# mkofinas/aether

Hardware: AMD Instinct MI355X
Metric: edge-messages/sec (forward, electrostatic N=20 batch=128 per GPU) (higher is better)
Workload: dtype f32; 1 GPU; electrostatic-2d-N20-B128; num_dims=2, nodes_per_graph=20, graphs_per_gpu=128, edges_per_gpu=48640, hidden=64, launch=hipgraph (10 steps per replay), parallelism=graphs sharded over 1 rank(s), no forward collective

## Files before the change

aether_amd/csrc/common.h:

```cpp
#pragma once
#include <hip/hip_runtime.h>
#include <cstdint>
#include <type_traits>
#include "../../include/aether_hip.h"

namespace {

typedef float f32x4 __attribute__((ext_vector_type(4)));
typedef float f32x2 __attribute__((ext_vector_type(2)));

constexpr int H = AETHER_HIDDEN;
constexpr int LDW = H + 8;
constexpr int FPAD = 32;
constexpr int LDF = FPAD + 8;
constexpr int LDST = H + 4;
constexpr float PI_F = 3.14159274101257324f;
constexpr float TWO_PI_F = 6.28318548202514648f;
constexpr float EPS_F = 1e-7f;

__device__ __forceinline__ void lds_barrier() { asm volatile("s_waitcnt lgkmcnt(0)\n\ts_barrier" ::: "memory"); }

__device__ __forceinline__ f32x4 mfma16(float a, float b, f32x4 c) {
    return __builtin_amdgcn_mfma_f32_16x16x4f32(a, b, c, 0, 0, 0);
}
// ... 121 lines not shown
    }
    const int frag = (mb * KBN + kb) * 64 + m + 16 * qq;
    constexpr int TERM = MBN * KBN * 64;
    *reinterpret_cast<f16x4*>(img + (frag) * 4 + half * 2) = h;
    *reinterpret_cast<f16x4*>(img + (TERM + frag) * 4 + half * 2) = l;
}

__device__ __forceinline__ unsigned wave_max_bits(float m) {
    int v = __float_as_int(m);
#define AETHER_DPP_MAX(CTRL) { const int o = __builtin_amdgcn_update_dpp(0, v, CTRL, 0xf, 0xf, true); v = o > v ? o : v; }
    AETHER_DPP_MAX(0x111) AETHER_DPP_MAX(0x112) AETHER_DPP_MAX(0x114) AETHER_DPP_MAX(0x118) AETHER_DPP_MAX(0x142) AETHER_DPP_MAX(0x143)
#undef AETHER_DPP_MAX
    return (unsigned)__builtin_amdgcn_readlane(v, 63);
}
__device__ __forceinline__ unsigned wave_max_exponent(float m) { return (wave_max_bits(m) >> 23) & 255u; }
struct SplitScale { bool on; float s, inv_s; };
__device__ __forceinline__ float absmax4(float m, const f32x4 v) {
#ifdef AETHER_SPLIT_PARENT_FORMS
    return fmaxf(fmaxf(m, fmaxf(fabsf(v[0]), fabsf(v[1]))), fmaxf(fabsf(v[2]), fabsf(v[3])));
#else
    m = fmaxf(fmaxf(m, fabsf(v[0])), fabsf(v[1]));
    return fmaxf(fmaxf(m, fabsf(v[2])), fabsf(v[3]));
#endif
}
template <int N>
__device__ __forceinline__ SplitScale split_scale_of(const f32x4 (&act)[N]) {
    float m = 0.0f;
#pragma unroll
    for (int b = 0; b < N; ++b) m = absmax4(m, act[b]);
    const bool big = __builtin_amdgcn_ballot_w64(m >= 32768.0f) != 0ull;
    const bool some = __builtin_amdgcn_ballot_w64(m >= 0.015625f) != 0ull;
    const bool any = __builtin_amdgcn_ballot_w64(m > 0.0f) != 0ull;
    SplitScale r;
    r.on = big || (any && !some);
    r.s = 1.0f; r.inv_s = 1.0f;
    if (r.on) {
        const unsigned E = wave_max_exponent(m);
        int sh = 140 - (int)E;
        sh = sh > 40 ? 40 : (sh < -40 ? -40 : sh);
        r.s = __int_as_float((127 + sh) << 23);
        r.inv_s = __int_as_float((127 - sh) << 23);
    }
    return r;
}

template <int MBN, int KBN>
__device__ __forceinline__ void gemm_split_core(const f16x8* __restrict__ w, const f32x4 (&act)[2 * KBN], f32x4 (&acc)[MBN], int lane,
                                                f16x8 (&xh)[KBN], f16x8 (&xl)[KBN]) {
    constexpr int TERM = MBN * KBN * 64;
#pragma unroll
    for (int kb = 0; kb < KBN; ++kb) {
        split8(act[2 * kb], act[2 * kb + 1], xh[kb], xl[kb]);
#pragma unroll
        for (int mb = 0; mb < MBN; ++mb) {
            const int frag = (mb * KBN + kb) * 64 + lane;
            const f16x8 wh = w[frag], wl = w[TERM + frag];
            acc[mb] = __builtin_amdgcn_mfma_f32_16x16x32_f16(wl, xh[kb], acc[mb], 0, 0, 0);
            acc[mb] = __builtin_amdgcn_mfma_f32_16x16x32_f16(wh, xl[kb], acc[mb], 0, 0, 0);
            acc[mb] = __builtin_amdgcn_mfma_f32_16x16x32_f16(wh, xh[kb], acc[mb], 0, 0, 0);
        }
    }
}
template <int MBN, int KBN>
__device__ __forceinline__ SplitScale gemm_split_keep(const float* __restrict__ img, const f32x4 (&act)[2 * KBN], f32x4 (&acc)[MBN],
                                                      int lane, f16x8 (&xh)[KBN], f16x8 (&xl)[KBN]) {
    const SplitScale sc = split_scale_of(act);
    f32x4 x[2 * KBN];
#pragma unroll
    for (int b = 0; b < 2 * KBN; ++b) x[b] = act[b];
    if (sc.on) {
#pragma unroll
        for (int b = 0; b < 2 * KBN; ++b) x[b] = x[b] * sc.s;
#pragma unroll
        for (int mb = 0; mb < MBN; ++mb) acc[mb] = acc[mb] * sc.s;
    }
    gemm_split_core<MBN, KBN>(reinterpret_cast<const f16x8*>(img), x, acc, lane, xh, xl);
    if (sc.on) {
#pragma unroll
        for (int mb = 0; mb < MBN; ++mb) acc[mb] = acc[mb] * sc.inv_s;
    }
    return sc;
}
template <int MBN, int KBN>
__device__ __forceinline__ void gemm_split(const float* __restrict__ img, const f32x4 (&act)[2 * KBN], f32x4 (&acc)[MBN],
                                           int lane) {
    f16x8 xh[KBN], xl[KBN];
    (void)gemm_split_keep<MBN, KBN>(img, act, acc, lane, xh, xl);
}

template <int MBN, int KBN>
__device__ __forceinline__ void gemm_split_paired(const float* __restrict__ img, const f32x4 (&act)[2 * KBN], f32x4 (&acc)[MBN], int lane) {
    static_assert(MBN % 2 == 0, "row blocks go in pairs");
    constexpr int TERM = MBN * KBN * 64, NG = KBN * (MBN / 2);
    const f16x8* w = reinterpret_cast<const f16x8*>(img);
    const SplitScale sc = split_scale_of(act);
    f32x4 x[2 * KBN];
#pragma unroll
    for (int b = 0; b < 2 * KBN; ++b) x[b] = act[b];
    if (sc.on) {
#pragma unroll
        for (int b = 0; b < 2 * KBN; ++b) x[b] = x[b] * sc.s;
#pragma unroll
        for (int mb = 0; mb < MBN; ++mb) acc[mb] = acc[mb] * sc.s;
    }
    auto frag = [&](int g, int j, bool lo) -> f16x8 {
        const int kb = g / (MBN / 2), mb = 2 * (g % (MBN / 2)) + j;
        return w[(lo ? TERM : 0) + (mb * KBN + kb) * 64 + lane];
    };
    f16x8 xh[KBN], xl[KBN];
    f16x8 wl0 = frag(0, 0, true), wl1 = frag(0, 1, true), wh0 = frag(0, 0, false), wh1 = frag(0, 1, false);
    split8(x[0], x[1], xh[0], xl[0]);
#pragma unroll
    for (int g = 0; g < NG; ++g) {
        const int kb = g / (MBN / 2), m0 = 2 * (g % (MBN / 2)), m1 = m0 + 1;
        __builtin_amdgcn_sched_barrier(0);
        acc[m0] = __builtin_amdgcn_mfma_f32_16x16x32_f16(wl0, xh[kb], acc[m0], 0, 0, 0);
        acc[m1] = __builtin_amdgcn_mfma_f32_16x16x32_f16(wl1, xh[kb], acc[m1], 0, 0, 0);
        __builtin_amdgcn_sched_barrier(0);
        if (g + 1 < NG) { wl0 = frag(g + 1, 0, true); wl1 = frag(g + 1, 1, true); }
        if (g + 1 < NG && (g + 1) % (MBN / 2) == 0) split8(x[2 * (kb + 1)], x[2 * (kb + 1) + 1], xh[kb + 1], xl[kb + 1]);
        acc[m0] = __builtin_amdgcn_mfma_f32_16x16x32_f16(wh0, xl[kb], acc[m0], 0, 0, 0);
        acc[m1] = __builtin_amdgcn_mfma_f32_16x16x32_f16(wh1, xl[kb], acc[m1], 0, 0, 0);
        acc[m0] = __builtin_amdgcn_mfma_f32_16x16x32_f16(wh0, xh[kb], acc[m0], 0, 0, 0);
        acc[m1] = __builtin_amdgcn_mfma_f32_16x16x32_f16(wh1, xh[kb], acc[m1], 0, 0, 0);
        __builtin_amdgcn_sched_barrier(0);
        if (g + 1 < NG) { wh0 = frag(g + 1, 0, false); wh1 = frag(g + 1, 1, false); }
    }
    if (sc.on) {
#pragma unroll
        for (int mb = 0; mb < MBN; ++mb) acc[mb] = acc[mb] * sc.inv_s;
    }
}

template <int KBN>
__device__ __forceinline__ f32x4 gemm_split_regs(const f16x8 (&wh)[KBN], const f16x8 (&wl)[KBN], const f32x4 (&act)[2 * KBN], f32x4 acc) {
    const SplitScale sc = split_scale_of(act);
    f32x4 x[2 * KBN];
#pragma unroll
    for (int b = 0; b < 2 * KBN; ++b) x[b] = act[b];
    if (sc.on) {
#pragma unroll
        for (int b = 0; b < 2 * KBN; ++b) x[b] = x[b] * sc.s;
        acc = acc * sc.s;
    }
#pragma unroll
    for (int kb = 0; kb < KBN; ++kb) {
        f16x8 xh, xl;
        split8(x[2 * kb], x[2 * kb + 1], xh, xl);
        acc = __builtin_amdgcn_mfma_f32_16x16x32_f16(wl[kb], xh, acc, 0, 0, 0);
        acc = __builtin_amdgcn_mfma_f32_16x16x32_f16(wh[kb], xl, acc, 0, 0, 0);
        acc = __builtin_amdgcn_mfma_f32_16x16x32_f16(wh[kb], xh, acc, 0, 0, 0);
    }
    if (sc.on) acc = acc * sc.inv_s;
    return acc;
}
template <int MBN, int KBN>
__device__ __forceinline__ void load_split_frags(const float* __restrict__ img, int mb, int lane, f16x8 (&wh)[KBN], f16x8 (&wl)[KBN]) {
    const f16x8* w = reinterpret_cast<const f16x8*>(img) + __builtin_amdgcn_readfirstlane(mb) * (KBN * 64);
    constexpr int TERM = MBN * KBN * 64;
#pragma unroll
    for (int kb = 0; kb < KBN; ++kb) {
        wh[kb] = w[kb * 64 + lane];
        wl[kb] = w[TERM + kb * 64 + lane];
    }
}

template <int KBN, int BLK>
__device__ __forceinline__ void split_T_issue(unsigned base, u32x2 (&lo)[2], u32x2 (&hi)[2]) {
    constexpr int TERM_BYTES = 4 * KBN * 64 * 16, OB = 2 * KBN, mp = BLK / OB, ob = BLK % OB;
#pragma unroll
    for (int t = 0; t < 2; ++t)
        asm volatile("ds_read_b64_tr_b16 %0, %2 offset:%3\n\tds_read_b64_tr_b16 %1, %2 offset:%4"
                     : "=&v"(lo[t]), "=&v"(hi[t])
                     : "v"(base), "n"(t * TERM_BYTES + (((2 * mp) * KBN + (ob >> 1)) * 64) * 16 + (ob & 1) * 8),
                       "n"(t * TERM_BYTES + (((2 * mp + 1) * KBN + (ob >> 1)) * 64) * 16 + (ob & 1) * 8)
                     : "memory");
}
template <bool LAST>
__device__ __forceinline__ void split_T_consume(u32x2 (&lo)[2], u32x2 (&hi)[2], const f16x8 xh, const f16x8 xl, f32x4& acc) {
    if constexpr (LAST)
        asm volatile("s_waitcnt lgkmcnt(0)" : "+v"(lo[0]), "+v"(hi[0]), "+v"(lo[1]), "+v"(hi[1]));
    else
        asm volatile("s_waitcnt lgkmcnt(4)" : "+v"(lo[0]), "+v"(hi[0]), "+v"(lo[1]), "+v"(hi[1]));
    f16x8 w[2];
#pragma unroll
    for (int t = 0; t < 2; ++t) {
        const u32x4 v = {lo[t][0], lo[t][1], hi[t][0], hi[t][1]};
        w[t] = __builtin_bit_cast(f16x8, v);
    }
    const f16x8 wh = w[0], wl = w[1];
    acc = __builtin_amdgcn_mfma_f32_16x16x32_f16(wl, xh, acc, 0, 0, 0);
    acc = __builtin_amdgcn_mfma_f32_16x16x32_f16(wh, xl, acc, 0, 0, 0);
    acc = __builtin_amdgcn_mfma_f32_16x16x32_f16(wh, xh, acc, 0, 0, 0);
}
template <int KBN, int BLK>
__device__ __forceinline__ void split_T_step(unsigned base, u32x2 (&lo)[2][2], u32x2 (&hi)[2][2], const f16x8 (&xh)[2],
                                             const f16x8 (&xl)[2], f32x4 (&acc)[2 * KBN]) {
    constexpr int OB = 2 * KBN, NBLK = 2 * OB, mp = BLK / OB, ob = BLK % OB;
    if constexpr (BLK + 1 < NBLK) split_T_issue<KBN, BLK + 1>(base, lo[(BLK + 1) & 1], hi[(BLK + 1) & 1]);
    split_T_consume<BLK + 1 == NBLK>(lo[BLK & 1], hi[BLK & 1], xh[mp], xl[mp], acc[ob]);
    if constexpr (BLK + 1 < NBLK) split_T_step<KBN, BLK + 1>(base, lo, hi, xh, xl, acc);
}
template <int KBN>
__device__ __forceinline__ SplitScale gemm_split_T_keep(const float* __restrict__ img, const f32x4 (&act)[4], f32x4 (&acc)[2 * KBN],
                                                        int lane, f16x8 (&xh)[2], f16x8 (&xl)[2]) {
    const int g = lane >> 4, r = (lane & 15) >> 2, p = lane & 3;
    const unsigned base = (unsigned)(size_t)(__attribute__((address_space(3))) const char*)img + ((4 * g + r) + 16 * p) * 16;
    const SplitScale sc = split_scale_of(act);
    f32x4 x[4];
#pragma unroll
    for (int b = 0; b < 4; ++b) x[b] = act[b];
    if (sc.on) {
#pragma unroll
        for (int b = 0; b < 4; ++b) x[b] = x[b] * sc.s;
    }
    split8(x[0], x[1], xh[0], xl[0]);
    split8(x[2], x[3], xh[1], xl[1]);
    u32x2 lo[2][2], hi[2][2];
    split_T_issue<KBN, 0>(base, lo[0], hi[0]);
    split_T_step<KBN, 0>(base, lo, hi, xh, xl, acc);
    if (sc.on) {
#pragma unroll
        for (int ob = 0; ob < 2 * KBN; ++ob) acc[ob] = acc[ob] * sc.inv_s;
    }
    return sc;
}
template <int KBN>
__device__ __forceinline__ void gemm_split_T(const float* __restrict__ img, const f32x4 (&act)[4], f32x4 (&acc)[2 * KBN],
                                             int lane) {
    f16x8 xh[2], xl[2];
    (void)gemm_split_T_keep<KBN>(img, act, acc, lane, xh, xl);
}

template <int MBN, int KBN>
__device__ __forceinline__ void gemm_split_pieces(const float* __restrict__ img, const f16x8 (&xh)[KBN], const f16x8 (&xl)[KBN],
                                                  const SplitScale sc, f32x4 (&acc)[MBN], int lane) {
    constexpr int TERM = MBN * KBN * 64;
    const f16x8* w = reinterpret_cast<const f16x8*>(img);
    if (sc.on) {
#pragma unroll
        for (int mb = 0; mb < MBN; ++mb) acc[mb] = acc[mb] * own_reg(sc.s);
    }
#pragma unroll
    for (int kb = 0; kb < KBN; ++kb)
#pragma unroll
        for (int mb = 0; mb < MBN; ++mb) {
            const int frag = (mb * KBN + kb) * 64 + lane;
            const f16x8 wh = w[frag], wl = w[TERM + frag];
            acc[mb] = __builtin_amdgcn_mfma_f32_16x16x32_f16(wl, xh[kb], acc[mb], 0, 0, 0);
            acc[mb] = __builtin_amdgcn_mfma_f32_16x16x32_f16(wh, xl[kb], acc[mb], 0, 0, 0);
            acc[mb] = __builtin_amdgcn_mfma_f32_16x16x32_f16(wh, xh[kb], acc[mb], 0, 0, 0);
        }
    if (sc.on) {
#pragma unroll
        for (int mb = 0; mb < MBN; ++mb) acc[mb] = acc[mb] * own_reg(sc.inv_s);
    }
}
template <int KBN>
__device__ __forceinline__ SplitScale split_tile(const f32x4 (&act)[2 * KBN], f16x8 (&xh)[KBN], f16x8 (&xl)[KBN]) {
    const SplitScale sc = split_scale_of(act);
#pragma unroll
    for (int kb = 0; kb < KBN; ++kb) {
        if (sc.on) split8(act[2 * kb] * own_reg(sc.s), act[2 * kb + 1] * own_reg(sc.s), xh[kb], xl[kb]);
        else split8(act[2 * kb], act[2 * kb + 1], xh[kb], xl[kb]);
    }
    return sc;
}

constexpr int FB_RH = 2 * LDST;
constexpr int FB_PLANE = 16 * FB_RH;
static_assert(2 * FB_PLANE == 16 * LDST * 4, "the two pieces take the room of the fp32 rows");
template <int KBN>
__device__ __forceinline__ void fb_stage_pieces(float* arr, int i, int q, const f16x8 (&xh)[KBN], const f16x8 (&xl)[KBN]) {
    char* row = reinterpret_cast<char*>(arr) + i * FB_RH + 8 * q;
#pragma unroll
    for (int kb = 0; kb < KBN; ++kb) {
        const u32x4 h = __builtin_bit_cast(u32x4, xh[kb]), l = __builtin_bit_cast(u32x4, xl[kb]);
        *reinterpret_cast<u32x2*>(row + 64 * kb) = u32x2{h[0], h[1]};
        *reinterpret_cast<u32x2*>(row + 64 * kb + 32) = u32x2{h[2], h[3]};
        *reinterpret_cast<u32x2*>(row + FB_PLANE + 64 * kb) = u32x2{l[0], l[1]};
        *reinterpret_cast<u32x2*>(row + FB_PLANE + 64 * kb + 32) = u32x2{l[2], l[3]};
    }
}
__device__ __forceinline__ unsigned fb_tr_lane_offset(int lane) {
    const int q = lane >> 4, c = lane & 15;
    return (unsigned)((4 * q + (c >> 2)) * FB_RH + 8 * (c & 3));
}
__device__ __forceinline__ unsigned fb_lds_addr(const float* p) { return (unsigned)(size_t)(__attribute__((address_space(3))) const char*)p; }
__device__ __forceinline__ f16x8 fb_frag(const u32x2 v) { return __builtin_bit_cast(f16x8, u32x4{v[0], v[1], 0u, 0u}); }
#define FB_TR(dst, base, off) asm volatile("ds_read_b64_tr_b16 %0, %1 offset:%2" : "=&v"(dst) : "v"(base), "n"(off) : "memory")
__device__ __forceinline__ f16x8 fb_inc_frag(unsigned nib) {
    const unsigned lo = ((nib & 1u) | ((nib & 2u) << 15)) * 0x3C00u, hi = (((nib >> 2) & 1u) | ((nib & 8u) << 13)) * 0x3C00u;
    return __builtin_bit_cast(f16x8, u32x4{lo, hi, 0u, 0u});
}


__device__ __forceinline__ void stage_weight(float* lds, const float* __restrict__ w, int rows,
                                             int cols, int src_ld, int ldw) {
    for (int idx = threadIdx.x; idx < rows * ldw; idx += blockDim.x) {
        int r = idx / ldw, c = idx - r * ldw;
        lds[idx] = (c < cols) ? w[(size_t)r * src_ld + c] : 0.0f;
    }
}

template <int THREADS>
__device__ __forceinline__ void stage_weight64(float* lds, const float* __restrict__ w, int src_ld) {
// ... 118 lines not shown
```

aether_amd/csrc/fused.h:

```cpp
#pragma once
#include "common.h"
#include "fused_layout.h"
#include "fused_graph.h"
#include "fused_handoff.h"

namespace {

struct FusedDebug {
    float* nodeinfo; float* x[5]; float* e[4];
    float* n[4]; float* ps[3]; float* pr[3]; float* feat;
    int* flags;
    int* errword;
    const float* wimg;
    float* stamps;
    StepExtras step;
};
constexpr int FUSED_STAMPS = 512;

#ifdef AETHER_FUSED_STAMPS
#define FUSED_STAMP(id)                                                                          \
    do {                                                                                         \
        if (tid == 0 && blockIdx.x < 4096)                                                       \
            dbg.stamps[blockIdx.x * FUSED_STAMPS + (id)] = (float)(wall_clock64() - t_entry) * 0.01f; \
    } while (0)
// ... 569 lines not shown
                    for (int j = 0; j < 4; ++j) {
                        const int idx = base + 64 * j + lane, idc = idx < np * 16 ? idx : 0;
                        int slot = idc >> 4;
                        if (slot >= off) slot += n;
                        const int c = (idc & 15) * 4;
                        v[j] = __builtin_amdgcn_raw_buffer_load_b128(rsrc, (slot * H + c) * 4, 0, 16);
                        dst[j] = idx < np * 16 ? slot * LDW + c : -1;
                    }
                    __builtin_amdgcn_sched_barrier(0);
                    __builtin_amdgcn_s_waitcnt(0x0F70);
                    __builtin_amdgcn_sched_barrier(0);
#pragma unroll
                    for (int j = 0; j < 4; ++j) asm volatile("" :: "v"(v[j]));
#pragma unroll
                    for (int j = 0; j < 4; ++j) {
                        f32x4 f;
#pragma unroll
                        for (int r4 = 0; r4 < 4; ++r4) f[r4] = __uint_as_float(v[j][r4]);
                        if (dst[j] >= 0) st4(psb + dst[j], f);
                    }
                }
            } else
            for (int idx = lane; idx < np * 16; idx += 64) {
                int slot = idx >> 4;
                if (slot >= off) slot += n;
                const int c = (idx & 15) * 4;
                const u32x4 v = __builtin_amdgcn_raw_buffer_load_b128(rsrc, (slot * H + c) * 4, 0, 16);
                f32x4 f;
#pragma unroll
                for (int r4 = 0; r4 < 4; ++r4) f[r4] = __uint_as_float(v[r4]);
                st4(psb + slot * LDW + c, f);
            }
            asm volatile("s_waitcnt vmcnt(0) lgkmcnt(0)" ::: "memory");
            __builtin_amdgcn_wave_barrier();
            if (lane == 0) arrived[0] = layer;
            FUSED_WSTAMP(layer, 0, 7);
        };
        auto wait_partner_rows = [&]() {
            while (__builtin_amdgcn_readfirstlane(arrived[0]) < layer) __builtin_amdgcn_s_sleep(1);
            asm volatile("" ::: "memory");
        };
        auto early_product = [&]() {
            if (n_tiles > wave) {
                f32x4 g[4];
#pragma unroll
                for (int mb = 0; mb < 4; ++mb) g[mb] = f32x4{0.f, 0.f, 0.f, 0.f};
                gemm_split_paired<4, 2>(wA, e[0], g, lane);
#pragma unroll
                for (int mb = 0; mb < 4; ++mb) e[0][mb] = g[mb];
            }
        };
        auto front_act = [&](int r, f32x4 (&acc)[4], f32x4 (&h1)[4], bool last) {
            if (last) issue_loads(1);
#pragma unroll
            for (int mb = 0; mb < 4; ++mb) h1[mb] = silu4(acc[mb]);
        };
        auto back = [&](int r, const f32x4 (&h1)[4], bool last) {
            const int tile = NW * r + wave;
            f32x4 acc2[4];
            if (last) issue_loads(2);
#pragma unroll
            for (int mb = 0; mb < 4; ++mb) acc2[mb] = ld4(cb + CB_B2 + 16 * mb + 4 * q);
            gemm_split<4, 2>(wB, h1, acc2, lane);
            if (last) issue_loads(3);
#pragma unroll
            for (int mb = 0; mb < 4; ++mb) e[r][mb] = silu4(acc2[mb]);
            if constexpr (KEEP) {
                if (ke[r] >= 0 && dbg.e[layer - 1] != nullptr) {
#pragma unroll
                    for (int mb = 0; mb < 4; ++mb)
                        st4(dbg.e[layer - 1] + (int64_t)ke[r] * H + 16 * mb + 4 * q, e[r][mb]);
                }
            }
            float* wst = smem + L::WSTAGE + wave * (16 * LDST);
#pragma unroll
            for (int mb = 0; mb < 4; ++mb) st4(wst + i * LDST + 16 * mb + 4 * q, e[r][mb]);
            FUSED_WSTAMP(layer, r, 4);
            __builtin_amdgcn_wave_barrier();
            {
                float cv[16];
#pragma unroll
                for (int k = 0; k < 16; ++k) cv[k] = wst[k * LDST + lane];
                float* pcol = part + lane;
                unsigned ends = seg_ends[r];
                asm volatile("" : "+s"(ends));
                unsigned long long lo = (unsigned long long)seg_rows[r][0] | ((unsigned long long)seg_rows[r][1] << 32);
                unsigned long long hi = (unsigned long long)seg_rows[r][2] | ((unsigned long long)seg_rows[r][3] << 32);
                float sum = 0.0f;
#pragma unroll
                for (int k = 0; k < 16; ++k) {
                    sum += cv[k];
                    if ((ends >> k) & 1u) {
                        pcol[((unsigned)lo & 0xFFu) * LDW] = sum;
                        sum = 0.0f;
                        lo = (lo >> 8) | (hi << 56);
                        hi >>= 8;
                    }
                }
            }
            __builtin_amdgcn_wave_barrier();
            if (last) issue_loads(4);
        };
        {
            const int nvalid = n_tiles > wave ? (n_tiles - wave + NW - 1) / NW : 0;
            if (nvalid == 0) {
#pragma unroll
                for (int part = 1; part < 5; ++part) issue_loads(part);
            }
            const int recv_wave = GRAN && na >= 16 ? 0 : NW - 1;
            if (xch && wave == recv_wave) receive_partner_rows();
            bool have_rows = !xch || wave == recv_wave;
#pragma unroll
            for (int r = 0; r < ROUNDS; ++r) {
                if (r < nvalid) {
                    const bool last = r == nvalid - 1;
                    const bool partner_tile = xch && 16 * (NW * r + wave + 1) > na;
                    const bool late_tile = LATE && partner_tile;
                    FUSED_WSTAMP(layer, r, 0);
                    if constexpr (!LATE) {
                        if (partner_tile && !have_rows) {
                            wait_partner_rows();
                            have_rows = true;
                        }
                    }
                    FUSED_WSTAMP(layer, r, 1);
                    f32x4 acc[4], h1[4];
                    front_gemm(r, acc, last, late_tile);
                    FUSED_WSTAMP(layer, r, 3);
                    if (late_tile) {
                        if (!have_rows) {
                            wait_partner_rows();
                            have_rows = true;
                        }
                        FUSED_WSTAMP_ROWS(layer, r);
                        late_add(r, acc);
                    }
                    front_act(r, acc, h1, last);
                    FUSED_WSTAMP(layer, r, 2);
                    back(r, h1, last);
                    FUSED_WSTAMP(layer, r, 5);
                }
            }
        }
        FUSED_STAMP(4 + 8 * (layer - 1) + 2);
        lds_barrier();
        FUSED_STAMP(4 + 8 * (layer - 1) + 3);
        if (tid < FUSED_MAX_NODES * 16) {
            f32x4 sum = f32x4{0.f, 0.f, 0.f, 0.f};
            const int at0 = arange & 0xFF, at1 = (arange >> 8) & 0xFF, bt0 = (arange >> 16) & 0xFF, bt1 = arange >> 24;
            for (int t = at0; t < at1; ++t) sum += ld4(part + (aslot + t) * LDW + ac4);
            for (int t = bt0; t < bt1; ++t) sum += ld4(part + (aslot + t) * LDW + ac4);
            const f32x4 nv = ld4(xbuf + aslot * LDW + ac4) + sum / adeg;
            st4(nbuf + aslot * LDW + ac4, nv);
            if (keep && aslot < n) st4(dbg.n[layer - 1] + (int64_t)(nb + aslot) * H + ac4, nv);
        }
        __builtin_amdgcn_s_waitcnt(0x0F70);
        if (layer < 4) dma_images(layer + 1);
        lds_barrier();
        FUSED_STAMP(4 + 8 * (layer - 1) + 7);
        if (act3) {
            float* ubuf = smem + L::UBUF;
            const f32x4 bv = ld4(cb + CB_B3 + 16 * mb2 + 4 * q);
#pragma unroll
            for (int tn = 0; tn < 2; ++tn) {
                if (16 * tn < n) {
                    f32x4 nv[4];
#pragma unroll
                    for (int a = 0; a < 4; ++a) nv[a] = ld4(nbuf + (16 * tn + i) * LDW + 16 * a + 4 * q);
                    f32x4 acc;
                    if constexpr (NW == 12) {
                        const f16x8 wh2[2] = {wf_h[0], wf_h[1]}, wl2[2] = {wf_l[0], wf_l[1]};
                        acc = gemm_split_regs<2>(wh2, wl2, nv, bv);
                    } else {
                        acc = gemm_split_regs<2>(w3h, w3l, nv, bv);
                    }
                    st4(ubuf + (16 * tn + i) * LDU + 16 * mb2 + 4 * q, silu4(acc));
                }
            }
        }
        if constexpr (EARLY) {
            if (layer < 4) __builtin_amdgcn_s_waitcnt(0x0F70);
        }
        lds_barrier();
        FUSED_STAMP(4 + 8 * (layer - 1) + 4);
        if constexpr (EARLY) {
            if (layer < 4 && wave < 8) {
                FUSED_WSTAMP(layer + 1, 0, 8);
                early_product();
                FUSED_WSTAMP(layer + 1, 0, 9);
            }
        }

        if (do3) {
            const float* ubuf = smem + L::UBUF;
            f32x4 acc = ld4(cb + CB_B4 + 16 * mb3 + 4 * q);
#pragma unroll
            for (int hk = 0; hk < 2; ++hk) {
                f32x4 uv[4];
#pragma unroll
                for (int a = 0; a < 4; ++a) uv[a] = ld4(ubuf + (16 * tn3s + i) * LDU + 16 * (4 * hk + a) + 4 * q);
                if constexpr (NW == 12) {
                    const f16x8 wh2[2] = {wf_h[2 * hk], wf_h[2 * hk + 1]}, wl2[2] = {wf_l[2 * hk], wf_l[2 * hk + 1]};
                    acc = gemm_split_regs<2>(wh2, wl2, uv, acc);
                } else {
                    const f16x8 wh2[2] = {w4h[2 * hk], w4h[2 * hk + 1]}, wl2[2] = {w4l[2 * hk], w4l[2 * hk + 1]};
                    acc = gemm_split_regs<2>(wh2, wl2, uv, acc);
                }
            }
            acc += ld4(nbuf + (16 * tn3s + i) * LDW + 16 * mb3 + 4 * q);
            st4(xbuf + (16 * tn3s + i) * LDW + 16 * mb3 + 4 * q, acc);
            if (keep && 16 * tn3s + i < n)
                st4(dbg.x[layer] + (int64_t)(nb + 16 * tn3s + i) * H + 16 * mb3 + 4 * q, acc);
        }
        lds_barrier();
        FUSED_STAMP(4 + 8 * (layer - 1) + 5);
        if (layer < 4) {
            if constexpr (GRAN && !EARLY) __builtin_amdgcn_s_waitcnt(0x0F70);
            if constexpr (EARLY) {
                if (wave >= 8) {
                    FUSED_WSTAMP(layer + 1, 0, 8);
                    early_product();
                    FUSED_WSTAMP(layer + 1, 0, 9);
                }
            }
            if (16 * tn4 < n) {
                f32x4 xv[4];
#pragma unroll
                for (int a = 0; a < 4; ++a) xv[a] = ld4(xbuf + (16 * tn4 + i) * LDW + 16 * a + 4 * q);
                if (do_s) {
                    f32x4 accs;
                    if constexpr (NW == 12) {
                        const f16x8 wh2[2] = {wf_h[2], wf_h[3]}, wl2[2] = {wf_l[2], wf_l[3]};
                        accs = gemm_split_regs<2>(wh2, wl2, xv, f32x4{0.f, 0.f, 0.f, 0.f});
                    } else {
                        accs = gemm_split_regs<2>(wsh, wsl, xv, f32x4{0.f, 0.f, 0.f, 0.f});
                    }
                    if (16 * tn4 + i < n) {
                        st4(psb + (off + 16 * tn4 + i) * LDW + 16 * mb3 + 4 * q, accs);
                        float* gps = dbg.ps[layer - 1] + (int64_t)(nb + 16 * tn4 + i) * H + 16 * mb3 + 4 * q;
                        if (GRAN && wg.partner >= 0) {
                            gran_publish(gran_rsrc(dbg.flags, wg.goff, vb, nv), off + 16 * tn4 + i, 16 * mb3 + 4 * q, layer, accs);
                        } else if (wg.partner >= 0) {
                            typedef unsigned int u32x4 __attribute__((ext_vector_type(4)));
                            const auto rsrc = __builtin_amdgcn_make_buffer_rsrc(
                                dbg.ps[layer - 1] + (int64_t)nb * H, 0, n * H * 4, 0x00020000);
                            u32x4 bits;
#pragma unroll
                            for (int r4 = 0; r4 < 4; ++r4) bits[r4] = __float_as_uint(accs[r4]);
                            __builtin_amdgcn_raw_buffer_store_b128(bits, rsrc, ((16 * tn4 + i) * H + 16 * mb3 + 4 * q) * 4, 0, 16);
                        } else if (keep) {
                            st4(gps, accs);
                        }
                    }
                }
                if (do_r) {
                    f32x4 accr;
                    if constexpr (NW == 12) {
                        const f16x8 wh2[2] = {wf_h[2], wf_h[3]}, wl2[2] = {wf_l[2], wf_l[3]};
                        accr = gemm_split_regs<2>(wh2, wl2, xv, ld4(cb + CB_B1N + 16 * mb3 + 4 * q));
                    } else {
                        accr = gemm_split_regs<2>(wrh, wrl, xv, ld4(cb + CB_B1N + 16 * mb3 + 4 * q));
                    }
                    st4(prb + (16 * tn4 + i) * LDW + 16 * mb3 + 4 * q, accr);
                    if (keep && 16 * tn4 + i < n)
                        st4(dbg.pr[layer - 1] + (int64_t)(nb + 16 * tn4 + i) * H + 16 * mb3 + 4 * q, accr);
                }
            }
            if (!GRAN)
                asm volatile("s_waitcnt vmcnt(0)" ::: "memory");
            lds_barrier();
            if (!GRAN && wg.partner >= 0 && tid == 0)
                __hip_atomic_store(dbg.flags + blockIdx.x, layer, __ATOMIC_RELAXED, __HIP_MEMORY_SCOPE_AGENT);
            FUSED_STAMP(4 + 8 * (layer - 1) + 6);
        }
    }
    if (wg.partner >= 0 && tid == 0)
        __hip_atomic_store(dbg.flags + wg.partner, 0, __ATOMIC_RELAXED, __HIP_MEMORY_SCOPE_AGENT);
    if constexpr (GRAN) {
        if (wg.partner >= 0 && wave >= 8) gran_rearm(gran_rsrc(dbg.flags, wg.goff, vb, nv), nv, n, off, tid - 512, 256);
    }

    {
        float* o1 = smem + L::OBUF1;
        float* o2 = smem + L::OBUF2;
        const int mb = wave & 3, tn = NW == 12 ? 0 : (wave >> 2) & 1;
        const bool act = wave < 8 && 16 * tn < n;
        const bool act1 = NW == 12 ? wave < 4 && n > 0 : act;
        const bool act2 = NW == 12 ? wave >= 4 && wave < 8 && n > 0 : act;
        const float* cb = cblk;
        if (act1) {
            f32x4 xv[4];
#pragma unroll
            for (int a = 0; a < 4; ++a) xv[a] = ld4(xbuf + (16 * tn + i) * LDW + 16 * a + 4 * q);
            f32x4 acc;
            if constexpr (NW == 12) {
                const f16x8 wh2[2] = {wf_h[2], wf_h[3]}, wl2[2] = {wf_l[2], wf_l[3]};
                acc = gemm_split_regs<2>(wh2, wl2, xv, ld4(cb + CB_B1N + 16 * mb + 4 * q));
            } else {
                acc = gemm_split_regs<2>(wsh, wsl, xv, ld4(cb + CB_B1N + 16 * mb + 4 * q));
            }
            f32x4 v = silu4(acc);
            if constexpr (KEEP) {
                if (dbg.step.drop1 != nullptr && 16 * tn + i < n)
                    v = v * ld4(dbg.step.drop1 + (int64_t)(nb + 16 * tn + i) * H + 16 * mb + 4 * q);
            }
            st4(o1 + (16 * tn + i) * LDW + 16 * mb + 4 * q, v);
        }
        if constexpr (KEEP) {
            if (blockIdx.x == 0 && tid == 0 && dbg.step.dropword != nullptr) *dbg.step.dropword = dbg.step.drop1 != nullptr ? 1 : 0;
        }
        lds_barrier();
        if (act2) {
            f32x4 xv[4];
#pragma unroll
            for (int a = 0; a < 4; ++a) xv[a] = ld4(o1 + (16 * tn + i) * LDW + 16 * a + 4 * q);
            f32x4 acc;
            if constexpr (NW == 12) {
                const f16x8 wh2[2] = {wf_h[2], wf_h[3]}, wl2[2] = {wf_l[2], wf_l[3]};
                acc = gemm_split_regs<2>(wh2, wl2, xv, ld4(cb + CB_OB3 + 16 * mb + 4 * q));
            } else {
                acc = gemm_split_regs<2>(wrh, wrl, xv, ld4(cb + CB_OB3 + 16 * mb + 4 * q));
            }
            f32x4 v = silu4(acc);
            if constexpr (KEEP) {
                if (dbg.step.drop2 != nullptr && 16 * tn + i < n)
                    v = v * ld4(dbg.step.drop2 + (int64_t)(nb + 16 * tn + i) * H + 16 * mb + 4 * q);
            }
            st4(o2 + (16 * tn + i) * LDW + 16 * mb + 4 * q, v);
        }
        lds_barrier();
        if (wave < 2 && 16 * wave < n) {
            const int tn2 = wave;
            f32x4 y = f32x4{0.f, 0.f, 0.f, 0.f};
#pragma unroll
            for (int a = 0; a < 4; ++a) {
                const f32x4 w6v = ld4(cb + CB_OW6 + (i < D ? i : D - 1) * H + 16 * a + 4 * q);
                const f32x4 xv = ld4(o2 + (16 * tn2 + i) * LDW + 16 * a + 4 * q);
#pragma unroll
                for (int b = 0; b < 4; ++b) y = mfma16(w6v[b], xv[b], y);
            }
            const int node = 16 * tn2 + i;
            if (q == 0 && node < n) {
                float yl[D];
#pragma unroll
                for (int d = 0; d < D; ++d) yl[d] = y[d] + cb[CB_OB6 + d];
                const float* ni = ninfo + (off + node) * 24;
#pragma unroll
                for (int a = 0; a < D; ++a) {
                    float s = 0.f;
#pragma unroll
                    for (int b = 0; b < D; ++b) s += ni[NI::R + a * D + b] * yl[b];
                    float xn = ni[NI::P + a] + s;
                    if (arrived[1]) xn = __builtin_nanf("");
                    out[(int64_t)(nb + node) * D + a] = xn;
                    if (dbg.step.vel_out)
                        dbg.step.vel_out[(int64_t)(nb + node) * D + a] = (xn - ni[NI::P + a]) / dbg.step.dt;
                }
            }
        }
    }
    FUSED_STAMP(40);
#ifdef AETHER_FUSED_STAMPS
    if (tid == 0 && blockIdx.x < 4096)
        dbg.stamps[blockIdx.x * FUSED_STAMPS + 41] = (float)(__builtin_amdgcn_s_memtime() - c_entry);
#endif
}

}
```

aether_amd/csrc/fused_layout.h:

```cpp
#pragma once
#include "common.h"

namespace {

constexpr int FUSED_MAX_NODES = 32;
constexpr int FUSED_MAX_EDGES = 384;
constexpr int FUSED_MAX_TILES = FUSED_MAX_EDGES / 16;
constexpr int LDU = 2 * H + 8;

constexpr int FUSED_WIMG = SPLIT_WIMG;
constexpr int FUSED_CBLK = 768;
constexpr int CB_B1 = 0;
constexpr int CB_B2 = 64;
constexpr int CB_B3 = 128;
constexpr int CB_B4 = 256;
constexpr int CB_B1N = 320;
constexpr int CB_OB3 = 384;
constexpr int CB_OB6 = 448;
constexpr int CB_OW6 = 512;
template <int NW, int ROUNDS> struct FusedLds {
    static constexpr int WSZ = FUSED_WIMG;
    static constexpr int WA = 0;
    static constexpr int WB = WA + WSZ;
    static constexpr int CBLK = WB + WSZ;
    static constexpr int XBUF = CBLK + 2 * FUSED_CBLK;
    static constexpr int NBUF = XBUF + FUSED_MAX_NODES * LDW;
    static constexpr int PS = NBUF + FUSED_MAX_NODES * LDW;
    static constexpr int PR = PS + FUSED_MAX_NODES * LDW;
    static constexpr int NINFO = PR + FUSED_MAX_NODES * LDW;
    static constexpr int PART_ROWS = ROUNDS == 3 ? FUSED_MAX_NODES + FUSED_MAX_TILES : 2 * FUSED_MAX_NODES + 16;
    static constexpr int PART = NINFO + FUSED_MAX_NODES * 24;
    static constexpr int ARRIVED = PART + PART_ROWS * LDW;
    static constexpr int SCRATCH = ARRIVED + 4;
    static constexpr int FEAT_ROWS = 16 * (ROUNDS < 2 ? ROUNDS : 2);
    static constexpr int SCRATCH_SIZE =
        NW * FEAT_ROWS * LDF > NW * 16 * LDST ? NW * FEAT_ROWS * LDF : NW * 16 * LDST;
    static constexpr int TOTAL = SCRATCH + SCRATCH_SIZE;
    static constexpr int FIELD_Z = SCRATCH;
    static constexpr int FIELD_H1 = FIELD_Z + FUSED_MAX_NODES * 24;
    static constexpr int FIELD_H2 = FIELD_H1 + FUSED_MAX_NODES * 32;
    static constexpr int FIELD_F = FIELD_H2 + FUSED_MAX_NODES * 32;
    static constexpr int FIELD_W = FIELD_F + FUSED_MAX_NODES * 4;
    static constexpr int FW0 = FIELD_W;
    static constexpr int FW2 = FW0 + 32 * 22;
    static constexpr int FW4 = FW2 + 32 * 32;
    static constexpr int FB = FW4 + 3 * 32;
    static constexpr int FEMB = FB + 68;
    static constexpr int FIELD_END = FEMB + 48;
    static constexpr int FEAT = SCRATCH;
    static constexpr int WSTAGE = SCRATCH;
    static constexpr int UBUF = SCRATCH;
    static constexpr int OBUF1 = SCRATCH;
    static constexpr int OBUF2 = SCRATCH + FUSED_MAX_NODES * LDW;
    static_assert(FIELD_END <= TOTAL, "field scratch");
    static_assert(UBUF + FUSED_MAX_NODES * LDU <= TOTAL, "ubuf");
    static_assert(OBUF2 + FUSED_MAX_NODES * LDW <= TOTAL, "obuf");
    static_assert(TOTAL * 4 <= 160 * 1024, "LDS budget");
};

constexpr int FUSED_NIMG_W3 = 2 * 8 * 2 * 64 * 4, FUSED_NIMG_W4 = 2 * 4 * 4 * 64 * 4, FUSED_NIMG_WS = 2 * 4 * 2 * 64 * 4;
constexpr int FUSED_NIMG_LAYER = FUSED_NIMG_W3 + FUSED_NIMG_W4 + 2 * FUSED_NIMG_WS;
constexpr int FUSED_WIMG_SET = 8 * FUSED_WIMG + 4 * FUSED_NIMG_LAYER + 4 * FUSED_CBLK;
constexpr int FUSED_SPLIT_BLOCKS = 8 + 4 * 6 + 1;
__device__ __host__ constexpr int fused_wimg_offset(int layer, int which) { return ((layer - 1) * 2 + which) * FUSED_WIMG; }
__device__ __host__ constexpr int fused_nimg_offset(int layer, int which) {
    return 8 * FUSED_WIMG + (layer - 1) * FUSED_NIMG_LAYER +
           (which == 0 ? 0 : which == 1 ? FUSED_NIMG_W3 : which == 2 ? FUSED_NIMG_W3 + FUSED_NIMG_W4 : FUSED_NIMG_W3 + FUSED_NIMG_W4 + FUSED_NIMG_WS);
}
__device__ __host__ constexpr int fused_cblk_offset(int layer) { return 8 * FUSED_WIMG + 4 * FUSED_NIMG_LAYER + (layer - 1) * FUSED_CBLK; }

__device__ __forceinline__ float fused_cblk_value(const AetherParams& P, int nd, int layer, int c) {
    if (c < CB_B2) return layer == 1 ? P.l1_msg_b0[c] : 0.0f;
    if (c < CB_B3) return (layer == 1 ? P.l1_msg_b2 : P.ln_msg_b2[layer - 2])[c - CB_B2];
    if (c < CB_B4) return (layer == 1 ? P.l1_upd_b0 : P.ln_upd_b0[layer - 2])[c - CB_B3];
    if (c < CB_B1N) return (layer == 1 ? P.l1_upd_b2 : P.ln_upd_b2[layer - 2])[c - CB_B4];
    if (c < CB_OB3) return (layer < 4 ? P.ln_msg_b0[layer - 1] : P.out_b0)[c - CB_B1N];
    if (layer < 4) return 0.0f;
    if (c < CB_OB6) return P.out_b3[c - CB_OB3];
    if (c < CB_OB6 + 4) return c - CB_OB6 < nd ? P.out_b6[c - CB_OB6] : 0.0f;
    if (c >= CB_OW6 && c < CB_OW6 + nd * H) return P.out_w6[c - CB_OW6];
    return 0.0f;
}

__device__ __forceinline__ void split_weights_block(const AetherParams& P, int f1, int nd, float* __restrict__ wimg, int block, int tid) {
    if (block == FUSED_SPLIT_BLOCKS - 1) {
        for (int idx = tid; idx < 4 * FUSED_CBLK; idx += 512)
            wimg[fused_cblk_offset(1) + idx] = fused_cblk_value(P, nd, idx / FUSED_CBLK + 1, idx % FUSED_CBLK);
        return;
    }
    if (block >= 8) {
        const int nbk = block - 8, layer = nbk / 6 + 1, part = nbk % 6;
        if (part < 2) {
            const float* w3 = layer == 1 ? P.l1_upd_w0 : P.ln_upd_w0[layer - 2];
            float* img = wimg + fused_nimg_offset(layer, 0);
#pragma unroll
            for (int j = 0; j < 2; ++j) {
                const int idx = tid + 512 * j, rr = 64 * part + (idx >> 4), cc = (idx & 15) * 4;
                stage_split4<8, 2>(img, rr, cc, ld4(w3 + (size_t)rr * H + cc));
            }
        } else if (part < 4) {
            const float* w4 = layer == 1 ? P.l1_upd_w2 : P.ln_upd_w2[layer - 2];
            float* img = wimg + fused_nimg_offset(layer, 1);
#pragma unroll
            for (int j = 0; j < 2; ++j) {
                const int idx = tid + 512 * j, rr = 32 * (part - 2) + (idx >> 5), cc = (idx & 31) * 4;
                stage_split4<4, 4>(img, rr, cc, ld4(w4 + (size_t)rr * (2 * H) + cc));
            }
        } else {
            const float* src = layer < 4 ? P.ln_msg_w0[layer - 1] + (part == 4 ? 0 : H) : (part == 4 ? P.out_w0 : P.out_w3);
            const int ld = layer < 4 ? 3 * H : H;
            float* img = wimg + fused_nimg_offset(layer, part - 2);
#pragma unroll
            for (int j = 0; j < 2; ++j) {
                const int idx = tid + 512 * j, rr = idx >> 4, cc = (idx & 15) * 4;
                stage_split4<4, 2>(img, rr, cc, ld4(src + (size_t)rr * ld + cc));
            }
        }
        return;
    }
    const int layer = block / 2 + 1, which = block & 1;
    float* img = wimg + fused_wimg_offset(layer, which);
    if (which == 0 && layer == 1) {
        const int r = tid >> 3, c0 = (tid & 7) * 4;
        f32x4 v;
#pragma unroll
        for (int b = 0; b < 4; ++b) v[b] = c0 + b < f1 ? P.l1_msg_w0[r * f1 + c0 + b] : 0.0f;
        stage_split4<4, 1>(img, r, c0, v);
        return;
    }
    const float* src;
    int ld;
    if (which == 0) { src = P.ln_msg_w0[layer - 2] + 2 * H; ld = 3 * H; }
    else { src = layer == 1 ? P.l1_msg_w2 : P.ln_msg_w2[layer - 2]; ld = H; }
#pragma unroll
    for (int j = 0; j < 2; ++j) {
        const int idx = tid + 512 * j, rr = idx >> 4, cc = (idx & 15) * 4;
        stage_split4<4, 2>(img, rr, cc, ld4(src + (size_t)rr * ld + cc));
    }
}

}
```

Measured before the change: 6.009 billion edge-messages/s.

## Pre-split node activations into f16 hi/lo pieces once for reuse across GEMM waves

For the 12-wave config, producers of node activations (aggregated n, update hidden u, new x, output hidden) now write f16 hi/lo split fragments into dedicated LDS regions in MFMA operand order, plus a per-wave range flag word. Consumer GEMMs load the pre-split fragments directly instead of each wave reloading fp32 rows and re-splitting, and fall back to the scaled split path when the flags indicate out-of-range magnitudes. This cuts redundant LDS reads and split arithmetic at the cost of extra LDS footprint, extra stores, ballot work, and a uniform branch per GEMM. It also drops the second tn tile in the update GEMM under NW==12, which assumes at most 16 nodes per tile.

```diff
diff --git a/aether_amd/csrc/common.h b/aether_amd/csrc/common.h
--- a/aether_amd/csrc/common.h
+++ b/aether_amd/csrc/common.h
@@ -297,6 +297,51 @@
         acc = __builtin_amdgcn_mfma_f32_16x16x32_f16(wh[kb], xh, acc, 0, 0, 0);
     }
     if (sc.on) acc = acc * sc.inv_s;
+    return acc;
+}
+constexpr int SPLIT_PIECES = 2 * 2 * 64 * 4;
+__device__ __forceinline__ void pieces_store(float* __restrict__ pieces, int i, int q, int mb, const f32x4 v) {
+    f16x4 h, l;
+#pragma unroll
+    for (int p = 0; p < 2; ++p) {
+        f16x2 a, b;
+        split_pair(f32x2{v[2 * p], v[2 * p + 1]}, a, b);
+        h[2 * p] = a[0]; h[2 * p + 1] = a[1];
+        l[2 * p] = b[0]; l[2 * p + 1] = b[1];
+    }
+    const int at = ((mb >> 1) * 64 + i + 16 * q) * 4 + (mb & 1) * 2;
+    *reinterpret_cast<f16x4*>(pieces + at) = h;
+    *reinterpret_cast<f16x4*>(pieces + SPLIT_PIECES / 2 + at) = l;
+}
+__device__ __forceinline__ void range_word_store(float* __restrict__ slot, float m, int lane) {
+    const unsigned big = __builtin_amdgcn_ballot_w64(m >= 32768.0f) != 0ull;
+    const unsigned some = __builtin_amdgcn_ballot_w64(m >= 0.015625f) != 0ull;
+    const unsigned any = __builtin_amdgcn_ballot_w64(m > 0.0f) != 0ull;
+    if (lane == 0) *reinterpret_cast<unsigned*>(slot) = big | some << 1 | any << 2;
+}
+__device__ __forceinline__ f32x4 gemm_pieces_regs(const f16x8 (&wh)[2], const f16x8 (&wl)[2], const float* __restrict__ pieces,
+                                                  const float* __restrict__ words, const float* __restrict__ rows, int lane, f32x4 acc) {
+    const f16x8* pc = reinterpret_cast<const f16x8*>(pieces);
+    const u32x4 w = *reinterpret_cast<const u32x4*>(words);
+    f16x8 xh[2], xl[2];
+#pragma unroll
+    for (int kb = 0; kb < 2; ++kb) {
+        xh[kb] = pc[kb * 64 + lane];
+        xl[kb] = pc[128 + kb * 64 + lane];
+    }
+    const unsigned f = __builtin_amdgcn_readfirstlane(w[0] | w[1] | w[2] | w[3]);
+    if (__builtin_expect((f & 1u) || ((f & 4u) && !(f & 2u)), 0)) {
+        f32x4 act[4];
+#pragma unroll
+        for (int a = 0; a < 4; ++a) act[a] = ld4(rows + 16 * a);
+        return gemm_split_regs<2>(wh, wl, act, acc);
+    }
+#pragma unroll
+    for (int kb = 0; kb < 2; ++kb) {
+        acc = __builtin_amdgcn_mfma_f32_16x16x32_f16(wl[kb], xh[kb], acc, 0, 0, 0);
+        acc = __builtin_amdgcn_mfma_f32_16x16x32_f16(wh[kb], xl[kb], acc, 0, 0, 0);
+        acc = __builtin_amdgcn_mfma_f32_16x16x32_f16(wh[kb], xh[kb], acc, 0, 0, 0);
+    }
     return acc;
 }
 template <int MBN, int KBN>
diff --git a/aether_amd/csrc/fused.h b/aether_amd/csrc/fused.h
--- a/aether_amd/csrc/fused.h
+++ b/aether_amd/csrc/fused.h
@@ -745,6 +745,12 @@
             for (int t = bt0; t < bt1; ++t) sum += ld4(part + (aslot + t) * LDW + ac4);
             const f32x4 nv = ld4(xbuf + aslot * LDW + ac4) + sum / adeg;
             st4(nbuf + aslot * LDW + ac4, nv);
+            if constexpr (NW == 12) {
+                if (wave < 4) {
+                    pieces_store(smem + L::NPC, aslot, tid & 3, (tid & 15) >> 2, nv);
+                    range_word_store(smem + L::PFLAG + wave, absmax4(0.0f, nv), lane);
+                }
+            }
             if (keep && aslot < n) st4(dbg.n[layer - 1] + (int64_t)(nb + aslot) * H + ac4, nv);
         }
         __builtin_amdgcn_s_waitcnt(0x0F70);
@@ -755,19 +761,21 @@
             float* ubuf = smem + L::UBUF;
             const f32x4 bv = ld4(cb + CB_B3 + 16 * mb2 + 4 * q);
 #pragma unroll
-            for (int tn = 0; tn < 2; ++tn) {
+            for (int tn = 0; tn < (NW == 12 ? 1 : 2); ++tn) {
                 if (16 * tn < n) {
-                    f32x4 nv[4];
-#pragma unroll
-                    for (int a = 0; a < 4; ++a) nv[a] = ld4(nbuf + (16 * tn + i) * LDW + 16 * a + 4 * q);
-                    f32x4 acc;
                     if constexpr (NW == 12) {
                         const f16x8 wh2[2] = {wf_h[0], wf_h[1]}, wl2[2] = {wf_l[0], wf_l[1]};
-                        acc = gemm_split_regs<2>(wh2, wl2, nv, bv);
+                        const f32x4 uv = silu4(gemm_pieces_regs(wh2, wl2, smem + L::NPC, smem + L::PFLAG, nbuf + i * LDW + 4 * q, lane, bv));
+                        st4(ubuf + i * LDU + 16 * mb2 + 4 * q, uv);
+                        pieces_store(smem + L::UPC + (mb2 >> 2) * SPLIT_PIECES, i, q, mb2 & 3, uv);
+                        range_word_store(smem + L::PFLAG + 4 + mb2, absmax4(0.0f, uv), lane);
                     } else {
-                        acc = gemm_split_regs<2>(w3h, w3l, nv, bv);
-                    }
-                    st4(ubuf + (16 * tn + i) * LDU + 16 * mb2 + 4 * q, silu4(acc));
+                        f32x4 nv[4];
+#pragma unroll
+                        for (int a = 0; a < 4; ++a) nv[a] = ld4(nbuf + (16 * tn + i) * LDW + 16 * a + 4 * q);
+                        const f32x4 acc = gemm_split_regs<2>(w3h, w3l, nv, bv);
+                        st4(ubuf + (16 * tn + i) * LDU + 16 * mb2 + 4 * q, silu4(acc));
+                    }
                 }
             }
         }
@@ -789,19 +797,24 @@
             f32x4 acc = ld4(cb + CB_B4 + 16 * mb3 + 4 * q);
 #pragma unroll
             for (int hk = 0; hk < 2; ++hk) {
-                f32x4 uv[4];
-#pragma unroll
-                for (int a = 0; a < 4; ++a) uv[a] = ld4(ubuf + (16 * tn3s + i) * LDU + 16 * (4 * hk + a) + 4 * q);
                 if constexpr (NW == 12) {
                     const f16x8 wh2[2] = {wf_h[2 * hk], wf_h[2 * hk + 1]}, wl2[2] = {wf_l[2 * hk], wf_l[2 * hk + 1]};
-                    acc = gemm_split_regs<2>(wh2, wl2, uv, acc);
+                    acc = gemm_pieces_regs(wh2, wl2, smem + L::UPC + hk * SPLIT_PIECES, smem + L::PFLAG + 4 + 4 * hk,
+                                           ubuf + i * LDU + 64 * hk + 4 * q, lane, acc);
                 } else {
+                    f32x4 uv[4];
+#pragma unroll
+                    for (int a = 0; a < 4; ++a) uv[a] = ld4(ubuf + (16 * tn3s + i) * LDU + 16 * (4 * hk + a) + 4 * q);
                     const f16x8 wh2[2] = {w4h[2 * hk], w4h[2 * hk + 1]}, wl2[2] = {w4l[2 * hk], w4l[2 * hk + 1]};
                     acc = gemm_split_regs<2>(wh2, wl2, uv, acc);
                 }
             }
             acc += ld4(nbuf + (16 * tn3s + i) * LDW + 16 * mb3 + 4 * q);
             st4(xbuf + (16 * tn3s + i) * LDW + 16 * mb3 + 4 * q, acc);
+            if constexpr (NW == 12) {
+                pieces_store(smem + L::XPC, i, q, mb3, acc);
+                range_word_store(smem + L::PFLAG + 12 + mb3, absmax4(0.0f, acc), lane);
+            }
             if (keep && 16 * tn3s + i < n)
                 st4(dbg.x[layer] + (int64_t)(nb + 16 * tn3s + i) * H + 16 * mb3 + 4 * q, acc);
         }
@@ -818,13 +831,16 @@
             }
             if (16 * tn4 < n) {
                 f32x4 xv[4];
-#pragma unroll
-                for (int a = 0; a < 4; ++a) xv[a] = ld4(xbuf + (16 * tn4 + i) * LDW + 16 * a + 4 * q);
+                if constexpr (NW != 12) {
+#pragma unroll
+                    for (int a = 0; a < 4; ++a) xv[a] = ld4(xbuf + (16 * tn4 + i) * LDW + 16 * a + 4 * q);
+                }
                 if (do_s) {
                     f32x4 accs;
                     if constexpr (NW == 12) {
                         const f16x8 wh2[2] = {wf_h[2], wf_h[3]}, wl2[2] = {wf_l[2], wf_l[3]};
-                        accs = gemm_split_regs<2>(wh2, wl2, xv, f32x4{0.f, 0.f, 0.f, 0.f});
+                        accs = gemm_pieces_regs(wh2, wl2, smem + L::XPC, smem + L::PFLAG + 12, xbuf + i * LDW + 4 * q, lane,
+                                                f32x4{0.f, 0.f, 0.f, 0.f});
                     } else {
                         accs = gemm_split_regs<2>(wsh, wsl, xv, f32x4{0.f, 0.f, 0.f, 0.f});
                     }
@@ -850,7 +866,8 @@
                     f32x4 accr;
                     if constexpr (NW == 12) {
                         const f16x8 wh2[2] = {wf_h[2], wf_h[3]}, wl2[2] = {wf_l[2], wf_l[3]};
-                        accr = gemm_split_regs<2>(wh2, wl2, xv, ld4(cb + CB_B1N + 16 * mb3 + 4 * q));
+                        accr = gemm_pieces_regs(wh2, wl2, smem + L::XPC, smem + L::PFLAG + 12, xbuf + i * LDW + 4 * q, lane,
+                                                ld4(cb + CB_B1N + 16 * mb3 + 4 * q));
                     } else {
                         accr = gemm_split_regs<2>(wrh, wrl, xv, ld4(cb + CB_B1N + 16 * mb3 + 4 * q));
                     }
@@ -882,14 +899,15 @@
         const bool act2 = NW == 12 ? wave >= 4 && wave < 8 && n > 0 : act;
         const float* cb = cblk;
         if (act1) {
-            f32x4 xv[4];
-#pragma unroll
-            for (int a = 0; a < 4; ++a) xv[a] = ld4(xbuf + (16 * tn + i) * LDW + 16 * a + 4 * q);
             f32x4 acc;
             if constexpr (NW == 12) {
                 const f16x8 wh2[2] = {wf_h[2], wf_h[3]}, wl2[2] = {wf_l[2], wf_l[3]};
-                acc = gemm_split_regs<2>(wh2, wl2, xv, ld4(cb + CB_B1N + 16 * mb + 4 * q));
+                acc = gemm_pieces_regs(wh2, wl2, smem + L::XPC, smem + L::PFLAG + 12, xbuf + i * LDW + 4 * q, lane,
+                                       ld4(cb + CB_B1N + 16 * mb + 4 * q));
             } else {
+                f32x4 xv[4];
+#pragma unroll
+                for (int a = 0; a < 4; ++a) xv[a] = ld4(xbuf + (16 * tn + i) * LDW + 16 * a + 4 * q);
                 acc = gemm_split_regs<2>(wsh, wsl, xv, ld4(cb + CB_B1N + 16 * mb + 4 * q));
             }
             f32x4 v = silu4(acc);
@@ -898,20 +916,25 @@
                     v = v * ld4(dbg.step.drop1 + (int64_t)(nb + 16 * tn + i) * H + 16 * mb + 4 * q);
             }
             st4(o1 + (16 * tn + i) * LDW + 16 * mb + 4 * q, v);
+            if constexpr (NW == 12) {
+                pieces_store(smem + L::OPC, i, q, mb, v);
+                range_word_store(smem + L::PFLAG + 16 + mb, absmax4(0.0f, v), lane);
+            }
         }
         if constexpr (KEEP) {
             if (blockIdx.x == 0 && tid == 0 && dbg.step.dropword != nullptr) *dbg.step.dropword = dbg.step.drop1 != nullptr ? 1 : 0;
         }
         lds_barrier();
         if (act2) {
-            f32x4 xv[4];
-#pragma unroll
-            for (int a = 0; a < 4; ++a) xv[a] = ld4(o1 + (16 * tn + i) * LDW + 16 * a + 4 * q);
             f32x4 acc;
             if constexpr (NW == 12) {
                 const f16x8 wh2[2] = {wf_h[2], wf_h[3]}, wl2[2] = {wf_l[2], wf_l[3]};
-                acc = gemm_split_regs<2>(wh2, wl2, xv, ld4(cb + CB_OB3 + 16 * mb + 4 * q));
+                acc = gemm_pieces_regs(wh2, wl2, smem + L::OPC, smem + L::PFLAG + 16, o1 + i * LDW + 4 * q, lane,
+                                       ld4(cb + CB_OB3 + 16 * mb + 4 * q));
             } else {
+                f32x4 xv[4];
+#pragma unroll
+                for (int a = 0; a < 4; ++a) xv[a] = ld4(o1 + (16 * tn + i) * LDW + 16 * a + 4 * q);
                 acc = gemm_split_regs<2>(wrh, wrl, xv, ld4(cb + CB_OB3 + 16 * mb + 4 * q));
             }
             f32x4 v = silu4(acc);
diff --git a/aether_amd/csrc/fused_layout.h b/aether_amd/csrc/fused_layout.h
--- a/aether_amd/csrc/fused_layout.h
+++ b/aether_amd/csrc/fused_layout.h
@@ -52,6 +52,12 @@
     static constexpr int UBUF = SCRATCH;
     static constexpr int OBUF1 = SCRATCH;
     static constexpr int OBUF2 = SCRATCH + FUSED_MAX_NODES * LDW;
+    static constexpr int NPC = SCRATCH + (LDU > 2 * LDW ? LDU : 2 * LDW) * FUSED_MAX_NODES;
+    static constexpr int UPC = NPC + SPLIT_PIECES;
+    static constexpr int XPC = UPC + 2 * SPLIT_PIECES;
+    static constexpr int OPC = XPC + SPLIT_PIECES;
+    static constexpr int PFLAG = OPC + SPLIT_PIECES;
+    static_assert(NW != 12 || (NPC >= OBUF2 + FUSED_MAX_NODES * LDW && NPC >= UBUF + FUSED_MAX_NODES * LDU && PFLAG + 5 * 4 <= TOTAL && NPC % 4 == 0), "operand pieces");
     static_assert(FIELD_END <= TOTAL, "field scratch");
     static_assert(UBUF + FUSED_MAX_NODES * LDU <= TOTAL, "ubuf");
     static_assert(OBUF2 + FUSED_MAX_NODES * LDW <= TOTAL, "obuf");
```

After: 6.334 billion edge-messages/s, median of 6. 5.4% higher.
